# PKU-EPIC/PartManip

Hardware: AMD Instinct MI355X
Metric: PPO env-steps/sec (whole node), 4096 envs x 1024-pt clouds (higher is better)
Workload: dtype f32

## Files before the change

partmanip_amd/csrc/pointnet_enc_screen.h:

```cpp
#pragma once

typedef __bf16 ps_bf16x8 __attribute__((ext_vector_type(8)));

#define PS_LDP (PN_C2 + 8)
#define PS_CAP 128
#define PS_NW 8
#define PS_P3 (16 * 16 * 64 * 8)
#define PS_OFF_P3H 0
#define PS_OFF_P3L (2 * PS_P3)
#define PS_OFF_W3 (4 * PS_P3 + 8192)
#define PS_OFF_EPS (PS_OFF_W3 + PN_C3 * PN_C2 * 4)
#define PS_PACKED_BYTES (PS_OFF_EPS + PN_C3 * 4)
#ifndef PS_ABLATE
#define PS_ABLATE 0
#endif
#ifndef PS_SCHED_DEFAULT
#define PS_SCHED_DEFAULT 0
#endif

extern "C" size_t pm_pointnet_packed_screen_bytes(void) { return PS_PACKED_BYTES; }

__device__ __forceinline__ unsigned ps_cvt_pk(float a, float b) {
    unsigned r;
    asm("v_cvt_pk_bf16_f32 %0, %1, %2" : "=v"(r) : "v"(a), "v"(b));
    return r;
}
__device__ __forceinline__ void ps_split(float x, unsigned short& hi, unsigned short& lo) {
    const unsigned h = ps_cvt_pk(x, 0.f) & 0xffffu;
    const float xh = __uint_as_float(h << 16);
    hi = (unsigned short)h;
    lo = (unsigned short)(ps_cvt_pk(x - xh, 0.f) & 0xffffu);
}

__global__ __launch_bounds__(256) void ps_pack_kernel(const float* __restrict__ W3, const float* __restrict__ b3,
                                                       unsigned char* __restrict__ packed) {
    const int i = blockIdx.x * 256 + threadIdx.x;
    if (i >= PS_P3) return;
    unsigned short* Ph = (unsigned short*)(packed + PS_OFF_P3H);
    unsigned short* Pl = (unsigned short*)(packed + PS_OFF_P3L);
    float* Wr = (float*)(packed + PS_OFF_W3);
    const int e = i & 7, lane = (i >> 3) & 63, li = lane & 31, lq = lane >> 5, step = (i >> 9) & 15, nb = i >> 13;
    unsigned short h, l;
    ps_split(W3[(nb * 32 + li) * PN_C2 + step * 16 + lq * 8 + e], h, l);
    Ph[i] = h;
    Pl[i] = l;
    Wr[i] = W3[i];
    if (i < 4096) ((unsigned short*)(packed + 4 * PS_P3))[i] = 0;
    if (i < PN_C3) {
        double L = 0.0;
        for (int k = 0; k < PN_C2; ++k) L += fabs((double)W3[i * PN_C2 + k]);
        const double ed = (0x1p-16 + 2048.0 * 0x1p-24) * (L + fabs((double)b3[i])) * (1.0 + 0x1p-10);
        float ef = (float)ed;
        if ((double)ef < ed) ef = __uint_as_float(__float_as_uint(ef) + 1);
        ((float*)(packed + PS_OFF_EPS))[i] = ef;
    }
}

extern "C" int pm_pointnet_pack_weights_screen(const float* W3, const float* b3, void* packed, void* stream) {
    PM_REQUIRE(W3 && b3 && packed);
    if (((uintptr_t)packed & 15) != 0) return PM_EALIGN;
    hipLaunchKernelGGL(ps_pack_kernel, dim3(PS_P3 / 256), dim3(256), 0, pm_stream(stream), W3, b3, (unsigned char*)packed);
    PM_CHECK_LAUNCH();
    return PM_OK;
}

#define PS_MFMA(a, b, c) __builtin_amdgcn_mfma_f32_32x32x16_bf16((a), (b), (c), 0, 0, 0)
__device__ __forceinline__ ps_bf16x8 ps_bf(const uint4& v) { return *(const ps_bf16x8*)&v; }

__device__ __forceinline__ void ps_stream(const unsigned short* __restrict__ Ah, const unsigned short* __restrict__ Al,
                                          const uint4* __restrict__ Bh, const uint4* __restrict__ Bl, f32x16 (&acc)[2][2]) {
    uint4 bh0[2], bl0[2], bh1[2], bl1[2];
#pragma unroll
    for (int nb = 0; nb < 2; ++nb) {
        bh0[nb] = Bh[(size_t)(nb * 16) * 64];
        bl0[nb] = Bl[(size_t)(nb * 16) * 64];
    }
#define PS_STEP(S_, BHC, BLC, BHN, BLN)                                                        \
    {                                                                                          \
        uint4 ah[2], al[2];                                                                    \
        _Pragma("unroll") for (int mb = 0; mb < 2; ++mb) {                                     \
            ah[mb] = *(const uint4*)(Ah + mb * 32 * PS_LDP + (S_) * 16);                       \
            al[mb] = *(const uint4*)(Al + mb * 32 * PS_LDP + (S_) * 16);                       \
        }                                                                                      \
        _Pragma("unroll") for (int nb = 0; nb < 2; ++nb) {    \
            BHN[nb] = Bh[(size_t)(nb * 16 + (S_) + 1) * 64];                                   \
            BLN[nb] = Bl[(size_t)(nb * 16 + (S_) + 1) * 64];                                   \
        }                                                                                      \
        __builtin_amdgcn_sched_barrier(0);                                                     \
        _Pragma("unroll") for (int nb = 0; nb < 2; ++nb)                                       \
            _Pragma("unroll") for (int mb = 0; mb < 2; ++mb) {                                 \
                acc[mb][nb] = PS_MFMA(ps_bf(ah[mb]), ps_bf(BHC[nb]), acc[mb][nb]);             \
                acc[mb][nb] = PS_MFMA(ps_bf(ah[mb]), ps_bf(BLC[nb]), acc[mb][nb]);             \
                acc[mb][nb] = PS_MFMA(ps_bf(al[mb]), ps_bf(BHC[nb]), acc[mb][nb]);             \
            }                                                                                  \
        __builtin_amdgcn_sched_barrier(0);                                                     \
    }
#pragma unroll 1
    for (int s = 0; s < 16; s += 2) {
        PS_STEP(s, bh0, bl0, bh1, bl1)
        PS_STEP(s + 1, bh1, bl1, bh0, bl0)
    }
#undef PS_STEP
}

template <int SCHED>
__device__ __forceinline__ bool ps_late_wave(int wave) { return SCHED == 1 && __builtin_amdgcn_readfirstlane(wave) >= 4; }

template <int NT>
__device__ __forceinline__ void ps_copy_h2(const float* __restrict__ H, float* __restrict__ dst, int tid) {
#pragma unroll 2
    for (int i = 0; i < PN_TM * PN_C2 / 4 / NT; ++i) {
        const int q = tid + NT * i, row = q >> 6, c4 = q & 63;
        const f32x4 v = *(const f32x4*)(H + row * PN_LD2 + 4 * c4);
        *(f32x4*)(dst + row * PN_C2 + 4 * c4) = v;
    }
}

static_assert(PN_TM * PN_MAXC == PS_NW * 64, "one staged slot per thread");
__device__ __forceinline__ float ps_point_load(const float* __restrict__ xb, int tile, int C, int tid) {
    const int p = tid >> 3, d = tid & 7;
    return d < C ? xb[(tile * PN_TM + p) * C + d] : 0.f;
}
__device__ __forceinline__ void ps_point_store(float v, int sub_mean, const float (&cen)[3], int tid, float* __restrict__ Xs) {
    const int d = tid & 7;
    if (sub_mean && d < 3) v -= cen[d];
    Xs[tid] = v;
}

#ifdef PS_PROFILE
__device__ unsigned long long ps_prof[4 * 16 * PS_NW * 16];
extern "C" int pm_debug_ps_prof_read(void* dst) {
    return hipMemcpyFromSymbol(dst, HIP_SYMBOL(ps_prof), sizeof(ps_prof)) == hipSuccess ? 0 : 1;
}
#define PS_STAMP(i)                                                                                         \
    if (b < 4 && tile < 16 && lane0 == 0) ps_prof[((b * 16 + tile) * PS_NW + wave) * 16 + (i)] = __builtin_readcyclecounter()
#else
#define PS_STAMP(i)
#endif

template <int CT, int SCHED>
__global__ __launch_bounds__(PS_NW * 64, 2) void pn_fwd_screen_kernel(
    const float* __restrict__ x, long ldx, int P, int C, int sub_mean, const float* __restrict__ W1,
    const float* __restrict__ b1, const float* __restrict__ b2, const float* __restrict__ b3,
    const float* __restrict__ packed, const unsigned char* __restrict__ packed_s, int max_mean, float* __restrict__ feat,
    long ldf, int32_t* __restrict__ argmax, float* __restrict__ h2_save, unsigned long long* __restrict__ counters) {
    constexpr int NT = PS_NW * 64;
    __shared__ __attribute__((aligned(16))) float H[PN_TM * PN_LD2];
    __shared__ __attribute__((aligned(16))) unsigned short Hp[2 * PN_TM * PS_LDP];
    __shared__ __attribute__((aligned(16))) float Xs[PN_TM * PN_MAXC];
    __shared__ double red[16];
    __shared__ double cs[PN_C2];
    __shared__ int skey[PS_NW][PS_CAP];
    unsigned short* Hh = Hp;
    unsigned short* Hl = Hp + PN_TM * PS_LDP;

    const int b = blockIdx.x, tid = threadIdx.x, lane0 = tid & 63, wave = tid >> 6;
    const float* xb = x + (long)b * ldx;
    const float4* P2v = (const float4*)(packed + PN_P2_OFF);
    const float4* P3v = (const float4*)(packed + PN_P3_OFF);
    const uint4* S3h = (const uint4*)(packed_s + PS_OFF_P3H);
    const uint4* S3l = (const uint4*)(packed_s + PS_OFF_P3L);
    const float* W3r = (const float*)(packed_s + PS_OFF_W3);
    const float* epsg = (const float*)(packed_s + PS_OFF_EPS);

    float cen[3] = {0.f, 0.f, 0.f};
    if (sub_mean) cloud_centroid<NT>(xb, P, C, red, cen);

    float vmax = -INFINITY, pois = 0.f;
    int imax = 0;
    double csum = 0.0;

    const int li0 = lane0 & 31;
    const float b2r = b2[wave * 32 + li0];
    const float b3r[2] = {b3[(wave * 2 + 0) * 32 + li0], b3[(wave * 2 + 1) * 32 + li0]};
    const float epsr[2] = {epsg[(wave * 2 + 0) * 32 + li0], epsg[(wave * 2 + 1) * 32 + li0]};
    float w1r[4] = {0.f, 0.f, 0.f, 0.f}, b1r = 0.f;
    if constexpr (CT == 3 || CT == 4) layer1_row<CT>(W1, b1, w1r, b1r);

    const int ntiles = P / PN_TM;
    stage_points<PN_TM, NT>(xb, 0, C, sub_mean, cen, Xs);
    for (int tile = 0; tile < ntiles; ++tile) {
        int lane = lane0;
        asm volatile("" : "+v"(lane));
        const int li = lane & 31, lh = lane >> 5;
        PS_STAMP(0);
        __syncthreads();
        float xnext = 0.f;
        if (tile + 1 < ntiles) xnext = ps_point_load(xb, tile + 1, C, tid);
        if (!(PS_ABLATE & 1)) {
            if constexpr (CT == 3 || CT == 4) layer1_tile<CT, PN_TM, NT, true>(Xs, w1r, b1r, H);
            else layer1_tile<CT, PN_TM, NT, true>(Xs, W1, b1, C, H);
        }
        PS_STAMP(1);
        __syncthreads();
        {
            f32x16 acc2[2][1];
            zero_acc<2, 1>(acc2);
            if (PS_ABLATE & 2) {
#pragma unroll
                for (int mb = 0; mb < 2; ++mb)
#pragma unroll
                    for (int r = 0; r < 16; ++r)
                        acc2[mb][0][r] = H[(mb * 32 + (r & 3) + 8 * (r >> 2) + 4 * lh) * PN_LD1 + ((wave * 32 + li) & 127)];
            } else {
                layer2_mfma<2, 1>(H, P2v, wave, lane, acc2);
            }
            PS_STAMP(2);
            __syncthreads();
            PS_STAMP(3);
            const int col = wave * 32 + li;
            const float b2c = b2r;
            float ts = 0.f;
            const bool planes = !(PS_ABLATE & 8) || tile == 0;
            const bool odd = (lane & 1) != 0;
            unsigned* Hh2 = (unsigned*)(Hh + (odd ? PS_LDP : 0) + (col & ~1));
            unsigned* Hl2 = (unsigned*)(Hl + (odd ? PS_LDP : 0) + (col & ~1));
#pragma unroll
            for (int mb = 0; mb < 2; ++mb)
#pragma unroll
                for (int r = 0; r < 16; r += 2) {
                    const float z0 = acc2[mb][0][r] + b2c, z1 = acc2[mb][0][r + 1] + b2c;
                    f32x2 v2;
                    if (PS_ABLATE & 4) {
                        v2.x = z0;
                        v2.y = z1;
                    } else {
                        v2 = pm_tanh2(z0, z1);
                    }
                    const int row0 = mb * 32 + (r & 3) + 8 * (r >> 2) + 4 * lh;
                    H[row0 * PN_LD2 + col] = v2.x;
                    H[(row0 + 1) * PN_LD2 + col] = v2.y;
                    ts += v2.x;
                    ts += v2.y;
                    const float own = odd ? v2.y : v2.x, send = odd ? v2.x : v2.y;
                    const float recv = __int_as_float(__builtin_amdgcn_update_dpp(0, __float_as_int(send), 0xB1, 0xf, 0xf, false));
                    const float a = odd ? recv : own, c = odd ? own : recv;
                    unsigned h2w, l2w;
                    if (PS_ABLATE & 4) {
                        h2w = (__float_as_uint(a) >> 16) | (__float_as_uint(c) & 0xffff0000u);
                        l2w = 0;
                    } else {
                        h2w = ps_cvt_pk(a, c);
                        l2w = ps_cvt_pk(a - __uint_as_float(h2w << 16), c - __uint_as_float(h2w & 0xffff0000u));
                    }
                    if (planes) {
                        Hh2[row0 * (PS_LDP / 2)] = h2w;
                        Hl2[row0 * (PS_LDP / 2)] = l2w;
                    }
                }
            ts += __shfl_xor(ts, 32, 64);
            csum += (double)ts;
            if (tile + 1 < ntiles) ps_point_store(xnext, sub_mean, cen, tid, Xs);
        }
        PS_STAMP(4);
        __syncthreads();
        PS_STAMP(5);

        const bool copy = h2_save && !(PS_ABLATE & 128), late = ps_late_wave<SCHED>(wave);
        float* h2dst = copy ? h2_save + ((long)b * P + (long)tile * PN_TM) * PN_C2 : nullptr;
        if (copy && late) ps_copy_h2<NT>(H, h2dst, tid);

        f32x16 acc[2][2];
#pragma unroll
        for (int nb = 0; nb < 2; ++nb) {
            const float b3c = b3r[nb];
#pragma unroll
            for (int r = 0; r < 16; ++r) acc[0][nb][r] = acc[1][nb][r] = b3c;
        }
        if (PS_ABLATE & 16) {
#pragma unroll
            for (int nb = 0; nb < 2; ++nb)
#pragma unroll
                for (int mb = 0; mb < 2; ++mb)
#pragma unroll
                    for (int r = 0; r < 16; ++r)
                        acc[mb][nb][r] += H[(mb * 32 + (r & 3) + 8 * (r >> 2) + 4 * lh) * PN_LD2 + ((wave * 64 + nb * 32 + li) & 255)];
        } else {
            ps_stream(Hh + li * PS_LDP + lh * 8, Hl + li * PS_LDP + lh * 8, S3h + (size_t)(wave * 2 * 16) * 64 + lane,
                      S3l + (size_t)(wave * 2 * 16) * 64 + lane, acc);
        }
        PS_STAMP(6);

        unsigned msk[2];
        float tmax[2];
#if (PS_ABLATE & 32) && defined(__HIP_DEVICE_COMPILE__)
#pragma unroll
        for (int nb = 0; nb < 2; ++nb) {
#pragma unroll
            for (int mb = 0; mb < 2; ++mb) asm volatile("" ::"v"(acc[mb][nb]));
            msk[nb] = 0;
            tmax[nb] = 0.f;
        }
#else
#pragma unroll
        for (int nb = 0; nb < 2; ++nb) {
            float m = -INFINITY;
#pragma unroll
            for (int mb = 0; mb < 2; ++mb)
#pragma unroll
                for (int r = 0; r < 16; ++r) m = fmaxf(m, acc[mb][nb][r]);
            m = fmaxf(m, __shfl_xor(m, 32, 64));
            const float e = epsr[nb];
            const float vm = __shfl(vmax, nb * 32 + li, 64);
            const float thr = m - 2.f * e;
            unsigned k = 0;
#pragma unroll
            for (int mb = 0; mb < 2; ++mb)
#pragma unroll
                for (int r = 0; r < 16; ++r) {
                    const float z = acc[mb][nb][r];
                    const bool s = !(z < thr) && !(z + e <= vm);
                    k |= (s ? 1u : 0u) << (mb * 16 + r);
                }
            msk[nb] = k;
            tmax[nb] = m;
        }
#endif
        const int n = __popc(msk[0]) + __popc(msk[1]);
        int incl = n;
#pragma unroll
        for (int o = 1; o < 64; o <<= 1) {
            const int t = __shfl_up(incl, o, 64);
            if (lane >= o) incl += t;
        }
        const int total = __builtin_amdgcn_readlane(incl, 63);
        PS_STAMP(7);

        if (PS_ABLATE & 64) {
            vmax = fmaxf(vmax, lh ? tmax[1] : tmax[0]);
            if (counters && lane == 0) atomicAdd(counters + 0, (unsigned long long)total);
        } else if (total <= PS_CAP) {
            int off = incl - n;
#pragma unroll
            for (int nb = 0; nb < 2; ++nb) {
                unsigned m = msk[nb];
                while (m) {
                    const int bit = __ffs(m) - 1;
                    m &= m - 1;
                    const int row = (bit >> 4) * 32 + (bit & 3) + 8 * ((bit & 15) >> 2) + 4 * lh;
                    skey[wave][off++] = (row << 6) | (nb * 32 + li);
                }
            }
            __builtin_amdgcn_wave_barrier();
            const int j = lane & 7, g = lane >> 3;
            for (int e0 = 0; e0 < total; e0 += 8) {
                const int e = e0 + g;
                const int key = (e < total) ? skey[wave][e] : 0;
                const int row = key >> 6, cl = key & 63;
                const float* hp = H + row * PN_LD2 + 4 * j;
                const float* wp = W3r + (size_t)(wave * 64 + cl) * PN_C2 + 4 * j;
                float s = 0.f;
#pragma unroll
                for (int i = 0; i < 8; ++i) {
                    const float4 w = *(const float4*)(wp + 32 * i);
                    const float4 h = *(const float4*)(hp + 32 * i);
                    s = fmaf(w.x, h.x, s);
                    s = fmaf(w.y, h.y, s);
                    s = fmaf(w.z, h.z, s);
                    s = fmaf(w.w, h.w, s);
                }
                s += __shfl_xor(s, 4, 64);
                s += __shfl_xor(s, 2, 64);
                s += __shfl_xor(s, 1, 64);
                s += b3[wave * 64 + cl];
#pragma unroll
                for (int gg = 0; gg < 8; ++gg)
                    if (e0 + gg < total) {
                        const int kk = __builtin_amdgcn_readlane(key, gg * 8);
                        const float v = __int_as_float(__builtin_amdgcn_readlane(__float_as_int(s), gg * 8));
                        if ((kk & 63) == lane) {
                            const int p = tile * PN_TM + (kk >> 6);
                            if (!(fabsf(v) < INFINITY)) pois += v;
                            if (v > vmax || (v == vmax && p < imax)) {
                                vmax = v;
                                imax = p;
                            }
                        }
                    }
            }
            if (counters) {
                const unsigned long long h0 = __ballot(msk[0] != 0), h1 = __ballot(msk[1] != 0);
                if (lane == 0) {
                    atomicAdd(counters + 0, (unsigned long long)total);
                    atomicAdd(counters + 2, (unsigned long long)(__popc((unsigned)(h0 | (h0 >> 32))) + __popc((unsigned)(h1 | (h1 >> 32)))));
                }
            }
        } else {
#pragma unroll
            for (int nb = 0; nb < 2; ++nb) {
                const float b3c = b3r[nb];
#pragma unroll
                for (int r = 0; r < 16; ++r) acc[0][nb][r] = acc[1][nb][r] = b3c;
            }
            mfma_stream<2, 2, 32>(H + li * PN_LD2 + lh * 128, PN_LD2, P3v + (size_t)(wave * 2) * 32 * 64 + lane, acc);
#pragma unroll
            for (int nb = 0; nb < 2; ++nb) {
                float bv = -INFINITY, ps = 0.f;
                int bp = 0;
#pragma unroll
                for (int mb = 0; mb < 2; ++mb)
#pragma unroll
                    for (int r = 0; r < 16; ++r) {
                        const float v = acc[mb][nb][r];
                        if (!(fabsf(v) < INFINITY)) ps += v;
                        if (v > bv) {
                            bv = v;
                            bp = tile * PN_TM + mb * 32 + (r & 3) + 8 * (r >> 2) + 4 * lh;
                        }
                    }
                const float ov = __shfl_xor(bv, 32, 64), os = __shfl_xor(ps, 32, 64);
                const int op = __shfl_xor(bp, 32, 64);
                if (ov > bv || (ov == bv && op < bp)) {
                    bv = ov;
                    bp = op;
                }
                if (lh == nb) {
                    pois += ps + os;
                    if (bv > vmax || (bv == vmax && bp < imax)) {
                        vmax = bv;
                        imax = bp;
                    }
                }
            }
            if (counters && lane == 0) atomicAdd(counters + 1, 1ull);
        }
        PS_STAMP(8);
        if (copy && !late) ps_copy_h2<NT>(H, h2dst, tid);
        PS_STAMP(9);
    }
    if ((lane0 >> 5) == 0) cs[wave * 32 + lane0] = csum;
    __syncthreads();
    const int ch = tid;
    float v = vmax;
    if (pois != pois) v = pois;
    feat[(long)b * ldf + ch] = v;
    argmax[(long)b * PN_C3 + ch] = imax;
    if (max_mean) {
        const float* wr = W3r + (size_t)ch * PN_C2;
        double s = 0.0;
#pragma unroll 4
        for (int k = 0; k < PN_C2; k += 4) {
            const float4 w = *(const float4*)(wr + k);
            s = fma((double)w.x, cs[k], s);
            s = fma((double)w.y, cs[k + 1], s);
            s = fma((double)w.z, cs[k + 2], s);
            s = fma((double)w.w, cs[k + 3], s);
        }
        float mv = (float)(s / (double)P + (double)b3[ch]);
        if (pois != pois) mv = pois;
        feat[(long)b * ldf + PN_C3 + ch] = mv;
    }
}

extern "C" int pm_pointnet_enc_fwd_screen_sched_f32(const float* x, long ldx, int B, int P, int C, int sub_mean, const float* W1,
                                                    const float* b1, const float* b2, const float* b3, const float* packed,
                                                    const void* packed_screen, int max_mean, float* feat, long ldf,
                                                    int32_t* argmax, float* h2_save, unsigned long long* counters, int schedule,
                                                    void* stream) {
    PM_REQUIRE(x && W1 && b1 && b2 && b3 && packed && packed_screen && feat && argmax);
    PM_REQUIRE(schedule == 0 || schedule == 1);
    if (h2_save && ((uintptr_t)h2_save & 15) != 0) return PM_EALIGN;
    PM_REQUIRE(B > 0 && P > 0 && P % PN_TM == 0 && C >= 1 && C <= PN_MAXC && ldx >= (long)P * C);
    PM_REQUIRE(ldf >= PN_C3 * (max_mean ? 2 : 1));
    PM_REQUIRE(!sub_mean || C >= 3);
    if (((uintptr_t)packed & 15) != 0 || ((uintptr_t)packed_screen & 15) != 0 || ((uintptr_t)counters & 7) != 0) return PM_EALIGN;
#define PS_LAUNCH(CT, S)                                                                                              \
    hipLaunchKernelGGL((pn_fwd_screen_kernel<CT, S>), dim3(B), dim3(PS_NW * 64), 0, pm_stream(stream), x, ldx, P, C, sub_mean, \
                       W1, b1, b2, b3, packed, (const unsigned char*)packed_screen, max_mean, feat, ldf, argmax, h2_save,   \
                       counters)
    if (schedule == 0) {
        if (C == 3) PS_LAUNCH(3, 0);
        else if (C == 4) PS_LAUNCH(4, 0);
        else PS_LAUNCH(0, 0);
    } else {
        if (C == 3) PS_LAUNCH(3, 1);
        else if (C == 4) PS_LAUNCH(4, 1);
        else PS_LAUNCH(0, 1);
    }
#undef PS_LAUNCH
    PM_CHECK_LAUNCH();
    return PM_OK;
}

extern "C" int pm_pointnet_enc_fwd_screen_f32(const float* x, long ldx, int B, int P, int C, int sub_mean, const float* W1,
                                              const float* b1, const float* b2, const float* b3, const float* packed,
                                              const void* packed_screen, int max_mean, float* feat, long ldf,
                                              int32_t* argmax, float* h2_save, unsigned long long* counters, void* stream) {
    return pm_pointnet_enc_fwd_screen_sched_f32(x, ldx, B, P, C, sub_mean, W1, b1, b2, b3, packed, packed_screen, max_mean, feat,
                                                ldf, argmax, h2_save, counters, PS_SCHED_DEFAULT, stream);
}
```

Measured before the change: 33470.

## Replace split-bf16 triple-MFMA screen with single scaled-fp16 MFMA per tile

The layer-3 screening matmul previously split activations and weights into bf16 hi/lo planes and issued three MFMAs per step. It now packs each output row's weights as fp16 scaled by a per-row power of two and issues one fp16 MFMA per step. Bias and inverse scale are applied after accumulation, and the per-row error bound eps is recomputed for fp16 rounding. The activation lo-plane in LDS and its conversions are dropped, and the prefetch is deepened to three B steps ahead. Looser screening bounds can admit more candidates for exact rechecking, so the candidate buffer capacity is doubled.

```diff
diff --git a/partmanip_amd/csrc/pointnet_enc_screen.h b/partmanip_amd/csrc/pointnet_enc_screen.h
--- a/partmanip_amd/csrc/pointnet_enc_screen.h
+++ b/partmanip_amd/csrc/pointnet_enc_screen.h
@@ -1,16 +1,16 @@
 #pragma once
 
-typedef __bf16 ps_bf16x8 __attribute__((ext_vector_type(8)));
+typedef _Float16 ps_f16x8 __attribute__((ext_vector_type(8)));
 
 #define PS_LDP (PN_C2 + 8)
-#define PS_CAP 128
+#define PS_CAP 256
 #define PS_NW 8
 #define PS_P3 (16 * 16 * 64 * 8)
-#define PS_OFF_P3H 0
-#define PS_OFF_P3L (2 * PS_P3)
-#define PS_OFF_W3 (4 * PS_P3 + 8192)
+#define PS_OFF_P3 0
+#define PS_OFF_W3 (2 * PS_P3)
 #define PS_OFF_EPS (PS_OFF_W3 + PN_C3 * PN_C2 * 4)
-#define PS_PACKED_BYTES (PS_OFF_EPS + PN_C3 * 4)
+#define PS_OFF_INV (PS_OFF_EPS + PN_C3 * 4)
+#define PS_PACKED_BYTES (PS_OFF_INV + PN_C3 * 4)
 #ifndef PS_ABLATE
 #define PS_ABLATE 0
 #endif
@@ -22,84 +22,103 @@
 
 __device__ __forceinline__ unsigned ps_cvt_pk(float a, float b) {
     unsigned r;
-    asm("v_cvt_pk_bf16_f32 %0, %1, %2" : "=v"(r) : "v"(a), "v"(b));
+    asm("v_cvt_pk_f16_f32 %0, %1, %2" : "=v"(r) : "v"(a), "v"(b));
     return r;
 }
-__device__ __forceinline__ void ps_split(float x, unsigned short& hi, unsigned short& lo) {
-    const unsigned h = ps_cvt_pk(x, 0.f) & 0xffffu;
-    const float xh = __uint_as_float(h << 16);
-    hi = (unsigned short)h;
-    lo = (unsigned short)(ps_cvt_pk(x - xh, 0.f) & 0xffffu);
-}
-
-__global__ __launch_bounds__(256) void ps_pack_kernel(const float* __restrict__ W3, const float* __restrict__ b3,
-                                                       unsigned char* __restrict__ packed) {
-    const int i = blockIdx.x * 256 + threadIdx.x;
-    if (i >= PS_P3) return;
-    unsigned short* Ph = (unsigned short*)(packed + PS_OFF_P3H);
-    unsigned short* Pl = (unsigned short*)(packed + PS_OFF_P3L);
-    float* Wr = (float*)(packed + PS_OFF_W3);
-    const int e = i & 7, lane = (i >> 3) & 63, li = lane & 31, lq = lane >> 5, step = (i >> 9) & 15, nb = i >> 13;
-    unsigned short h, l;
-    ps_split(W3[(nb * 32 + li) * PN_C2 + step * 16 + lq * 8 + e], h, l);
-    Ph[i] = h;
-    Pl[i] = l;
-    Wr[i] = W3[i];
-    if (i < 4096) ((unsigned short*)(packed + 4 * PS_P3))[i] = 0;
-    if (i < PN_C3) {
-        double L = 0.0;
-        for (int k = 0; k < PN_C2; ++k) L += fabs((double)W3[i * PN_C2 + k]);
-        const double ed = (0x1p-16 + 2048.0 * 0x1p-24) * (L + fabs((double)b3[i])) * (1.0 + 0x1p-10);
+
+__global__ __launch_bounds__(PN_C2) void ps_pack_kernel(const float* __restrict__ W3, const float* __restrict__ b3,
+                                                         unsigned char* __restrict__ packed) {
+    __shared__ double Ls[PN_C2], Rs[PN_C2], Ss[PN_C2];
+    __shared__ float Ms[PN_C2];
+    const int c = blockIdx.x, k = threadIdx.x;
+    const float w = W3[c * PN_C2 + k];
+    const float aw = fabsf(w);
+    Ls[k] = (double)aw;
+    Ms[k] = aw < INFINITY ? aw : 0.f;
+    __syncthreads();
+    for (int o = PN_C2 / 2; o > 0; o >>= 1) {
+        if (k < o) {
+            Ls[k] += Ls[k + o];
+            Ms[k] = fmaxf(Ms[k], Ms[k + o]);
+        }
+        __syncthreads();
+    }
+    int ex = -200;
+    if (Ms[0] > 0.f) frexpf(Ms[0], &ex);
+    const int s = min(15 - ex, 126);
+    const float ws = ldexpf(w, s);
+    const _Float16 w16 = (_Float16)ws;
+    const float wf = (float)w16, d = fabsf(ws - wf);
+    Rs[k] = (double)(fabsf(wf) < 0x1p-14f ? fmaxf(fabsf(ws), d) : d);
+    Ss[k] = (double)fabsf(wf);
+    __syncthreads();
+    for (int o = PN_C2 / 2; o > 0; o >>= 1) {
+        if (k < o) {
+            Rs[k] += Rs[k + o];
+            Ss[k] += Ss[k + o];
+        }
+        __syncthreads();
+    }
+    const int nb = c >> 5, li = c & 31, step = k >> 4, lq = (k >> 3) & 1, e = k & 7;
+    ((_Float16*)(packed + PS_OFF_P3))[(((nb * 16 + step) * 64) + lq * 32 + li) * 8 + e] = w16;
+    ((float*)(packed + PS_OFF_W3))[c * PN_C2 + k] = w;
+    if (k == 0) {
+        const double ed = ((Rs[0] + 0x1p-12 * Ss[0]) * ldexp(1.0, -s) + 1024.0 * 0x1p-24 * (Ls[0] + fabs((double)b3[c]))) * (1.0 + 0x1p-10) + 0x1p-116;
         float ef = (float)ed;
         if ((double)ef < ed) ef = __uint_as_float(__float_as_uint(ef) + 1);
-        ((float*)(packed + PS_OFF_EPS))[i] = ef;
+        ((float*)(packed + PS_OFF_EPS))[c] = ef;
+        ((float*)(packed + PS_OFF_INV))[c] = ldexpf(1.f, -s);
     }
 }
 
 extern "C" int pm_pointnet_pack_weights_screen(const float* W3, const float* b3, void* packed, void* stream) {
     PM_REQUIRE(W3 && b3 && packed);
     if (((uintptr_t)packed & 15) != 0) return PM_EALIGN;
-    hipLaunchKernelGGL(ps_pack_kernel, dim3(PS_P3 / 256), dim3(256), 0, pm_stream(stream), W3, b3, (unsigned char*)packed);
+    hipLaunchKernelGGL(ps_pack_kernel, dim3(PN_C3), dim3(PN_C2), 0, pm_stream(stream), W3, b3, (unsigned char*)packed);
     PM_CHECK_LAUNCH();
     return PM_OK;
 }
 
-#define PS_MFMA(a, b, c) __builtin_amdgcn_mfma_f32_32x32x16_bf16((a), (b), (c), 0, 0, 0)
-__device__ __forceinline__ ps_bf16x8 ps_bf(const uint4& v) { return *(const ps_bf16x8*)&v; }
-
-__device__ __forceinline__ void ps_stream(const unsigned short* __restrict__ Ah, const unsigned short* __restrict__ Al,
-                                          const uint4* __restrict__ Bh, const uint4* __restrict__ Bl, f32x16 (&acc)[2][2]) {
-    uint4 bh0[2], bl0[2], bh1[2], bl1[2];
+#define PS_MFMA(a, b, c) __builtin_amdgcn_mfma_f32_32x32x16_f16((a), (b), (c), 0, 0, 0)
+__device__ __forceinline__ ps_f16x8 ps_h(const uint4& v) { return *(const ps_f16x8*)&v; }
+
+__device__ __forceinline__ void ps_stream(const unsigned short* __restrict__ A, const uint4* __restrict__ B, f32x16 (&acc)[2][2]) {
+    uint4 b0[2], b1[2], b2[2], b3[2], a0[2], a1[2];
 #pragma unroll
     for (int nb = 0; nb < 2; ++nb) {
-        bh0[nb] = Bh[(size_t)(nb * 16) * 64];
-        bl0[nb] = Bl[(size_t)(nb * 16) * 64];
-    }
-#define PS_STEP(S_, BHC, BLC, BHN, BLN)                                                        \
+        b0[nb] = B[(size_t)(nb * 16 + 0) * 64];
+        b1[nb] = B[(size_t)(nb * 16 + 1) * 64];
+        b2[nb] = B[(size_t)(nb * 16 + 2) * 64];
+    }
+#pragma unroll
+    for (int mb = 0; mb < 2; ++mb) a0[mb] = *(const uint4*)(A + mb * 32 * PS_LDP);
+#define PS_STEP(S_, AC, AN, BC, BN, PFA, PFB)                                                  \
     {                                                                                          \
-        uint4 ah[2], al[2];                                                                    \
-        _Pragma("unroll") for (int mb = 0; mb < 2; ++mb) {                                     \
-            ah[mb] = *(const uint4*)(Ah + mb * 32 * PS_LDP + (S_) * 16);                       \
-            al[mb] = *(const uint4*)(Al + mb * 32 * PS_LDP + (S_) * 16);                       \
+        if (PFA) {                                                                             \
+            _Pragma("unroll") for (int mb = 0; mb < 2; ++mb)                                   \
+                AN[mb] = *(const uint4*)(A + mb * 32 * PS_LDP + ((S_) + 1) * 16);              \
         }                                                                                      \
-        _Pragma("unroll") for (int nb = 0; nb < 2; ++nb) {    \
-            BHN[nb] = Bh[(size_t)(nb * 16 + (S_) + 1) * 64];                                   \
-            BLN[nb] = Bl[(size_t)(nb * 16 + (S_) + 1) * 64];                                   \
+        if (PFB) {                                                                             \
+            _Pragma("unroll") for (int nb = 0; nb < 2; ++nb)                                   \
+                BN[nb] = B[(size_t)(nb * 16 + (S_) + 3) * 64];                                 \
         }                                                                                      \
         __builtin_amdgcn_sched_barrier(0);                                                     \
         _Pragma("unroll") for (int nb = 0; nb < 2; ++nb)                                       \
-            _Pragma("unroll") for (int mb = 0; mb < 2; ++mb) {                                 \
-                acc[mb][nb] = PS_MFMA(ps_bf(ah[mb]), ps_bf(BHC[nb]), acc[mb][nb]);             \
-                acc[mb][nb] = PS_MFMA(ps_bf(ah[mb]), ps_bf(BLC[nb]), acc[mb][nb]);             \
-                acc[mb][nb] = PS_MFMA(ps_bf(al[mb]), ps_bf(BHC[nb]), acc[mb][nb]);             \
-            }                                                                                  \
+            _Pragma("unroll") for (int mb = 0; mb < 2; ++mb)                                   \
+                acc[mb][nb] = PS_MFMA(ps_h(AC[mb]), ps_h(BC[nb]), acc[mb][nb]);                \
         __builtin_amdgcn_sched_barrier(0);                                                     \
     }
 #pragma unroll 1
-    for (int s = 0; s < 16; s += 2) {
-        PS_STEP(s, bh0, bl0, bh1, bl1)
-        PS_STEP(s + 1, bh1, bl1, bh0, bl0)
-    }
+    for (int s = 0; s < 12; s += 4) {
+        PS_STEP(s, a0, a1, b0, b3, 1, 1)
+        PS_STEP(s + 1, a1, a0, b1, b0, 1, 1)
+        PS_STEP(s + 2, a0, a1, b2, b1, 1, 1)
+        PS_STEP(s + 3, a1, a0, b3, b2, 1, 1)
+    }
+    PS_STEP(12, a0, a1, b0, b3, 1, 1)
+    PS_STEP(13, a1, a0, b1, b0, 1, 0)
+    PS_STEP(14, a0, a1, b2, b1, 1, 0)
+    PS_STEP(15, a1, a0, b3, b2, 0, 0)
 #undef PS_STEP
 }
 
@@ -146,22 +165,20 @@
     long ldf, int32_t* __restrict__ argmax, float* __restrict__ h2_save, unsigned long long* __restrict__ counters) {
     constexpr int NT = PS_NW * 64;
     __shared__ __attribute__((aligned(16))) float H[PN_TM * PN_LD2];
-    __shared__ __attribute__((aligned(16))) unsigned short Hp[2 * PN_TM * PS_LDP];
+    __shared__ __attribute__((aligned(16))) unsigned short Hh[PN_TM * PS_LDP];
     __shared__ __attribute__((aligned(16))) float Xs[PN_TM * PN_MAXC];
     __shared__ double red[16];
     __shared__ double cs[PN_C2];
     __shared__ int skey[PS_NW][PS_CAP];
-    unsigned short* Hh = Hp;
-    unsigned short* Hl = Hp + PN_TM * PS_LDP;
 
     const int b = blockIdx.x, tid = threadIdx.x, lane0 = tid & 63, wave = tid >> 6;
     const float* xb = x + (long)b * ldx;
     const float4* P2v = (const float4*)(packed + PN_P2_OFF);
     const float4* P3v = (const float4*)(packed + PN_P3_OFF);
-    const uint4* S3h = (const uint4*)(packed_s + PS_OFF_P3H);
-    const uint4* S3l = (const uint4*)(packed_s + PS_OFF_P3L);
+    const uint4* S3 = (const uint4*)(packed_s + PS_OFF_P3);
     const float* W3r = (const float*)(packed_s + PS_OFF_W3);
     const float* epsg = (const float*)(packed_s + PS_OFF_EPS);
+    const float* invg = (const float*)(packed_s + PS_OFF_INV);
 
     float cen[3] = {0.f, 0.f, 0.f};
     if (sub_mean) cloud_centroid<NT>(xb, P, C, red, cen);
@@ -174,6 +191,7 @@
     const float b2r = b2[wave * 32 + li0];
     const float b3r[2] = {b3[(wave * 2 + 0) * 32 + li0], b3[(wave * 2 + 1) * 32 + li0]};
     const float epsr[2] = {epsg[(wave * 2 + 0) * 32 + li0], epsg[(wave * 2 + 1) * 32 + li0]};
+    const float invr[2] = {invg[(wave * 2 + 0) * 32 + li0], invg[(wave * 2 + 1) * 32 + li0]};
     float w1r[4] = {0.f, 0.f, 0.f, 0.f}, b1r = 0.f;
     if constexpr (CT == 3 || CT == 4) layer1_row<CT>(W1, b1, w1r, b1r);
 
@@ -214,7 +232,6 @@
             const bool planes = !(PS_ABLATE & 8) || tile == 0;
             const bool odd = (lane & 1) != 0;
             unsigned* Hh2 = (unsigned*)(Hh + (odd ? PS_LDP : 0) + (col & ~1));
-            unsigned* Hl2 = (unsigned*)(Hl + (odd ? PS_LDP : 0) + (col & ~1));
 #pragma unroll
             for (int mb = 0; mb < 2; ++mb)
 #pragma unroll
@@ -235,18 +252,7 @@
                     const float own = odd ? v2.y : v2.x, send = odd ? v2.x : v2.y;
                     const float recv = __int_as_float(__builtin_amdgcn_update_dpp(0, __float_as_int(send), 0xB1, 0xf, 0xf, false));
                     const float a = odd ? recv : own, c = odd ? own : recv;
-                    unsigned h2w, l2w;
-                    if (PS_ABLATE & 4) {
-                        h2w = (__float_as_uint(a) >> 16) | (__float_as_uint(c) & 0xffff0000u);
-                        l2w = 0;
-                    } else {
-                        h2w = ps_cvt_pk(a, c);
-                        l2w = ps_cvt_pk(a - __uint_as_float(h2w << 16), c - __uint_as_float(h2w & 0xffff0000u));
-                    }
-                    if (planes) {
-                        Hh2[row0 * (PS_LDP / 2)] = h2w;
-                        Hl2[row0 * (PS_LDP / 2)] = l2w;
-                    }
+                    if (planes) Hh2[row0 * (PS_LDP / 2)] = ps_cvt_pk(a, c);
                 }
             ts += __shfl_xor(ts, 32, 64);
             csum += (double)ts;
@@ -261,12 +267,6 @@
         if (copy && late) ps_copy_h2<NT>(H, h2dst, tid);
 
         f32x16 acc[2][2];
-#pragma unroll
-        for (int nb = 0; nb < 2; ++nb) {
-            const float b3c = b3r[nb];
-#pragma unroll
-            for (int r = 0; r < 16; ++r) acc[0][nb][r] = acc[1][nb][r] = b3c;
-        }
         if (PS_ABLATE & 16) {
 #pragma unroll
             for (int nb = 0; nb < 2; ++nb)
@@ -274,10 +274,10 @@
                 for (int mb = 0; mb < 2; ++mb)
 #pragma unroll
                     for (int r = 0; r < 16; ++r)
-                        acc[mb][nb][r] += H[(mb * 32 + (r & 3) + 8 * (r >> 2) + 4 * lh) * PN_LD2 + ((wave * 64 + nb * 32 + li) & 255)];
+                        acc[mb][nb][r] = b3r[nb] + H[(mb * 32 + (r & 3) + 8 * (r >> 2) + 4 * lh) * PN_LD2 + ((wave * 64 + nb * 32 + li) & 255)];
         } else {
-            ps_stream(Hh + li * PS_LDP + lh * 8, Hl + li * PS_LDP + lh * 8, S3h + (size_t)(wave * 2 * 16) * 64 + lane,
-                      S3l + (size_t)(wave * 2 * 16) * 64 + lane, acc);
+            zero_acc<2, 2>(acc);
+            ps_stream(Hh + li * PS_LDP + lh * 8, S3 + (size_t)(wave * 2 * 16) * 64 + lane, acc);
         }
         PS_STAMP(6);
 
@@ -295,10 +295,14 @@
 #pragma unroll
         for (int nb = 0; nb < 2; ++nb) {
             float m = -INFINITY;
+            const float iv = invr[nb], b3c = b3r[nb];
 #pragma unroll
             for (int mb = 0; mb < 2; ++mb)
 #pragma unroll
-                for (int r = 0; r < 16; ++r) m = fmaxf(m, acc[mb][nb][r]);
+                for (int r = 0; r < 16; ++r) {
+                    if (!(PS_ABLATE & 16)) acc[mb][nb][r] = fmaf(acc[mb][nb][r], iv, b3c);
+                    m = fmaxf(m, acc[mb][nb][r]);
+                }
             m = fmaxf(m, __shfl_xor(m, 32, 64));
             const float e = epsr[nb];
             const float vm = __shfl(vmax, nb * 32 + li, 64);
```

Result: faster. 36220, median of 6 (+8.2%).
